# jianzhnie/ScaleRL

Hardware: NVIDIA H100
Metric: learner_frames_per_sec (higher is better)
Workload: dtype bf16

## Files before the change

scalerl_b200/csrc/encoder.cu:

```cuda
#include "encoder_problems.cuh"
#include "tma_problems.cuh"
#include "res_problems.cuh"
#include "enc_fused.cuh"
#include "kernels.h"
#include <stdio.h>
#include <stdlib.h>

namespace srl {

constexpr int PACK_BLOCKS_FK = 256, PACK_BLOCKS_FD = 256, PACK_BLOCKS_CONV = 288;
SRL_DEVINL void pack_store(bf16* __restrict__ out, bf16* __restrict__ out_lo, int64_t i, float v) {
  const bf16 hi = __float2bfloat16_rn(v);
  out[i] = hi;
  if (out_lo) out_lo[i] = __float2bfloat16_rn(v - __bfloat162float(hi));
}
SRL_DEVINL void pack_store2(bf16* __restrict__ out, bf16* __restrict__ out_lo, int64_t i, float v0, float v1) {
  const bf16 h0 = __float2bfloat16_rn(v0), h1 = __float2bfloat16_rn(v1);
  *reinterpret_cast<uint32_t*>(out + i) = pack_bf16x2(v0, v1);
  if (out_lo) *reinterpret_cast<uint32_t*>(out_lo + i) = pack_bf16x2(v0 - __bfloat162float(h0), v1 - __bfloat162float(h1));
}
__global__ void __launch_bounds__(256) pack_weights_kernel(ParamPtrs p, bf16* __restrict__ out, bf16* __restrict__ out_lo, int skip_w1k) {
  pdl_wait(2);
  __shared__ __align__(16) float tile[64 * 99];
  const int t = threadIdx.x, b = blockIdx.x;
  if (b < PACK_BLOCKS_FK) {
    const float4* src = reinterpret_cast<const float4*>(p.wf + (size_t)(2 * b) * 3136);
    float4 v[7];
#pragma unroll
    for (int u = 0; u < 7; ++u) { const int q = t + 256 * u; if (q < 1568) v[u] = __ldg(src + q); }
#pragma unroll
    for (int u = 0; u < 7; ++u) { const int q = t + 256 * u; if (q < 1568) *reinterpret_cast<float4*>(tile + 4 * q) = v[u]; }
    __syncthreads();
#pragma unroll 4
    for (int pp = t; pp < 2 * 1568; pp += 256) {
      const int r = pp >= 1568, k = 2 * (pp - r * 1568), hw = k >> 6, c = k & 63;
      const float* row = tile + r * 3136;
      pack_store2(out, out_lo, WPack::WFK + (int64_t)(2 * b + r) * 3136 + k, row[c * 49 + hw], row[(c + 1) * 49 + hw]);
    }
  } else if (b < PACK_BLOCKS_FK + PACK_BLOCKS_FD) {
    const int bb = b - PACK_BLOCKS_FK, j0 = (bb & 7) * 64, c0 = (bb >> 3) * 2;
    float2 v[13];
#pragma unroll
    for (int u = 0; u < 13; ++u) {
      const int q = t + 256 * u, jj = q / 49, e = q - jj * 49;
      if (q < 64 * 49) v[u] = __ldg(reinterpret_cast<const float2*>(p.wf + (size_t)(j0 + jj) * 3136 + c0 * 49 + 2 * e));
    }
#pragma unroll
    for (int u = 0; u < 13; ++u) {
      const int q = t + 256 * u, jj = q / 49, e = q - jj * 49;
      if (q < 64 * 49) { tile[jj * 99 + 2 * e] = v[u].x; tile[jj * 99 + 2 * e + 1] = v[u].y; }
    }
    __syncthreads();
    const int lane = t & 31, warp = t >> 5;
    for (int kk = warp; kk < 98; kk += 8) {
      const int cc = kk >= 49, hw = kk - cc * 49;
      pack_store2(out, out_lo, WPack::WFD + (int64_t)(hw * 64 + c0 + cc) * 512 + j0 + 2 * lane, tile[(2 * lane) * 99 + kk], tile[(2 * lane + 1) * 99 + kk]);
    }
  } else {
    const int bb = b - PACK_BLOCKS_FK - PACK_BLOCKS_FD;
    constexpr int64_t NCONV = WPack::WFK + (WPack::TOTAL - WPack::W3D);
    for (int64_t n = (int64_t)bb * 256 + t; n < NCONV; n += (int64_t)PACK_BLOCKS_CONV * 256) {
      const int64_t i = n < WPack::WFK ? n : n - WPack::WFK + WPack::W3D;
      float v;
      if (i < WPack::W2K) {
        if (skip_w1k) continue;
        const int e = (int)(i - WPack::W1K), co = e >> 8, k = e & 255, tap = k >> 6, q = k & 63;
        const int c = q >> 4, dy = (q >> 2) & 3, dx = q & 3, kh = 4 * (tap >> 1) + dy, kw = 4 * (tap & 1) + dx;
        v = p.w1[co * 256 + c * 64 + kh * 8 + kw];
      } else if (i < WPack::W3K) {
        const int e = (int)(i - WPack::W2K), co = e >> 9, k = e & 511, tap = k >> 5, c = k & 31;
        v = p.w2[((co * 32 + c) << 4) + tap];
      } else if (i < WPack::WFK) {
        const int e = (int)(i - WPack::W3K), co = e / 576, k = e - co * 576, tap = k >> 6, c = k & 63;
        v = p.w3[(co * 64 + c) * 9 + tap];
      } else if (i < WPack::W2D) {
        const int e = (int)(i - WPack::W3D), c = e / 576, k = e - c * 576, tap = k >> 6, co = k & 63;
        v = p.w3[(co * 64 + c) * 9 + tap];
      } else {
        const int e = (int)(i - WPack::W2D), cls = e >> 13, r = e & 8191, c = r >> 8, k = r & 255, tt = k >> 6, co = k & 63;
        const int kh = (cls >> 1) + 2 * (tt >> 1), kw = (cls & 1) + 2 * (tt & 1);
        v = p.w2[((co * 32 + c) << 4) + kh * 4 + kw];
      }
      pack_store(out, out_lo, i, v);
    }
  }
}

__global__ void __launch_bounds__(352) obs_s2d_kernel(const uint8_t* __restrict__ obs, bf16* __restrict__ xs, int frame_blocks,
                                                      const float* __restrict__ w1, bf16* __restrict__ w1k, bf16* __restrict__ w1k_lo) {
  pdl_wait(1);
  pdl_launch();
  if ((int)blockIdx.x >= frame_blocks) {
    const int e = ((int)blockIdx.x - frame_blocks) * 352 + (int)threadIdx.x;
    if (e < 32 * 256 && w1k) {
      const int co = e >> 8, k = e & 255, tap = k >> 6, q = k & 63;
      const int c = q >> 4, dy = (q >> 2) & 3, dx = q & 3, kh = 4 * (tap >> 1) + dy, kw = 4 * (tap & 1) + dx;
      pack_store(w1k, w1k_lo, e, __ldg(w1 + co * 256 + c * 64 + kh * 8 + kw));
    }
    return;
  }
  __shared__ uint32_t tile[21][16][21];
  const int n = blockIdx.x;
  const int t = threadIdx.x;
  if (t < 336) {
    const int g = t / 21, X = t - g * 21;
    const uint8_t* src = obs + (size_t)n * 28224 + (g >> 2) * 7056 + (g & 3) * 84;
#pragma unroll
    for (int y = 0; y < 21; ++y) tile[y][g][X] = __ldg(reinterpret_cast<const uint32_t*>(src + y * 336) + X);
  }
  __syncthreads();
  if (t < 336) {
    const int X = t >> 4, g = t & 15;
#pragma unroll
    for (int y = 0; y < 21; ++y) {
      const uint32_t w = tile[y][g][X];
      const float f0 = __uint_as_float(__byte_perm(w, 0x4B000000u, 0x7540)) - 8388608.f;
      const float f1 = __uint_as_float(__byte_perm(w, 0x4B000000u, 0x7541)) - 8388608.f;
      const float f2 = __uint_as_float(__byte_perm(w, 0x4B000000u, 0x7542)) - 8388608.f;
      const float f3 = __uint_as_float(__byte_perm(w, 0x4B000000u, 0x7543)) - 8388608.f;
      *reinterpret_cast<uint2*>(xs + (((size_t)n * 21 + y) * 21 + X) * 64 + g * 4) = make_uint2(pack_bf16x2(f0, f1), pack_bf16x2(f2, f3));
    }
  }
}

__global__ void __launch_bounds__(256) a3_transpose_kernel(const bf16* __restrict__ a3, bf16* __restrict__ a3t) {
  pdl_wait(53);
  __shared__ __align__(16) uint16_t tile[49 * 66];
  const int n = blockIdx.x, t = threadIdx.x;
  const uint4* src = reinterpret_cast<const uint4*>(a3 + (size_t)n * 3136);
  for (int q = t; q < 392; q += 256) {
    const uint4 v = __ldg(src + q);
    uint32_t* d = reinterpret_cast<uint32_t*>(tile + (q >> 3) * 66 + (q & 7) * 8);
    d[0] = v.x; d[1] = v.y; d[2] = v.z; d[3] = v.w;
  }
  __syncthreads();
  uint32_t* dst = reinterpret_cast<uint32_t*>(a3t + (size_t)n * 3136);
  for (int pp = t; pp < 1568; pp += 256) {
    const int o = 2 * pp, c0 = o / 49, h0 = o - c0 * 49, o1 = o + 1, c1 = o1 / 49, h1 = o1 - c1 * 49;
    dst[pp] = (uint32_t)tile[h0 * 66 + c0] | ((uint32_t)tile[h1 * 66 + c1] << 16);
  }
}
SRL_KSTAMP_SETTER(kstamp_set_encoder)

cudaError_t launch_a3_transpose(const bf16* a3, bf16* a3t, int frames, cudaStream_t st) {
  if (frames <= 0) return cudaSuccess;
  a3_transpose_kernel<<<frames, 256, 0, st>>>(a3, a3t);
  return cudaGetLastError();
}

cudaError_t launch_pack_weights(const ParamPtrs& p, bf16* wpack, cudaStream_t st, bf16* wpack_lo, bool skip_w1k) {
  pack_weights_kernel<<<PACK_BLOCKS_FK + PACK_BLOCKS_FD + PACK_BLOCKS_CONV, 256, 0, st>>>(p, wpack, wpack_lo, skip_w1k ? 1 : 0);
  return cudaGetLastError();
}

#define SRL_TRY(x) do { cudaError_t e_ = (x); if (e_ != cudaSuccess) return e_; } while (0)

static inline int cdiv(int a, int b) { return (a + b - 1) / b; }

typedef CUresult (*EncodeTiledFn)(CUtensorMap*, CUtensorMapDataType, cuuint32_t, void*, const cuuint64_t*, const cuuint64_t*,
                                  const cuuint32_t*, const cuuint32_t*, CUtensorMapInterleave, CUtensorMapSwizzle,
                                  CUtensorMapL2promotion, CUtensorMapFloatOOBfill);

static EncodeTiledFn encode_fn() {
  static EncodeTiledFn fn = nullptr;
  if (!fn) {
    void* f = nullptr;
    cudaDriverEntryPointQueryResult q;
    if (cudaGetDriverEntryPoint("cuTensorMapEncodeTiled", &f, cudaEnableDefault, &q) == cudaSuccess && q == cudaDriverEntryPointSuccess)
      fn = reinterpret_cast<EncodeTiledFn>(f);
  }
  return fn;
}

bool make_map(CUtensorMap* m, const void* base, int rank, const uint64_t* dims, const uint64_t* strides_elems, const uint32_t* box,
              bool swizzle64) {
  EncodeTiledFn fn = encode_fn();
  if (!fn) return false;
  cuuint64_t gd[5], gs[4];
  cuuint32_t bx[5], es[5];
  for (int i = 0; i < rank; ++i) { gd[i] = dims[i]; bx[i] = box[i]; es[i] = 1; }
  for (int i = 0; i + 1 < rank; ++i) gs[i] = strides_elems[i] * 2;
  return fn(m, CU_TENSOR_MAP_DATA_TYPE_BFLOAT16, (cuuint32_t)rank, const_cast<void*>(base), gd, gs, bx, es, CU_TENSOR_MAP_INTERLEAVE_NONE,
            swizzle64 ? CU_TENSOR_MAP_SWIZZLE_64B : CU_TENSOR_MAP_SWIZZLE_128B, CU_TENSOR_MAP_L2_PROMOTION_L2_128B,
            CU_TENSOR_MAP_FLOAT_OOB_FILL_NONE) == CUDA_SUCCESS;
}

struct MapBuilder {
  const char* failed = nullptr;
  bool lo = false, failed_lo = false;
  void operator()(CUtensorMap* m, const void* base, uint64_t inner, uint64_t rows, uint32_t box_inner, uint32_t box_rows, const char* name,
                  bool swizzle64 = false) {
    const uint64_t d[2] = {inner, rows}, s[1] = {inner};
    const uint32_t bx[2] = {box_inner, box_rows};
    if (!failed && !make_map(m, base, 2, d, s, bx, swizzle64)) { failed = name; failed_lo = lo; }
  }
};

static void build_operand_maps(MapBuilder& mk, const OperandTensors& b, uint64_t nf, uint64_t nb, OperandMaps* M) {
  mk(&M->a1p0_w, b.a1, 64, nf * 100, 64, RConv2Fwd::WROWS, "a1p0_w");
  mk(&M->a1p1_w, b.a1 + (size_t)nf * 100 * 64, 64, nf * 100, 64, RConv2Fwd::WROWS, "a1p1_w");
  mk(&M->a2_w, b.a2, 64, nf * 81, 64, RConv3Fwd::WROWS, "a2_w");
  mk(&M->da3g_w, b.da3, 64, nb * 81, 64, RConv3Dgrad::WROWS, "da3g_w");
  mk(&M->da3g_b, b.da3, 64, nb * 81, 64, 128, "da3g_b");
  mk(&M->da2g_w, b.da2, 64, nb * 100, 64, RConv2Dgrad::WROWS, "da2g_w");
  mk(&M->da2g_b, b.da2, 64, nb * 100, 64, 128, "da2g_b");
  mk(&M->da1g_b, b.da1, 32, nb * 441, 32, 128, "da1g_b", true);
  mk(&M->a3m128, b.a3, 3136, nf, 64, 128, "a3m128");
  mk(&M->a3m64, b.a3, 3136, nf, 64, 64, "a3m64");
  mk(&M->dhm128, b.dh, 512, nb, 64, 128, "dhm128");
  mk(&M->dhm64, b.dh, 512, nb, 64, 64, "dhm64");
  const bf16* w = b.wpack;
  mk(&M->w1k, w + WPack::W1K, 256, 32, 64, 32, "w1k");
  mk(&M->w2k, w + WPack::W2K, 512, 64, 64, 64, "w2k");
  mk(&M->w3k, w + WPack::W3K, 576, 64, 64, 64, "w3k");
  mk(&M->wfk, w + WPack::WFK, 3136, 512, 64, 64, "wfk");
  mk(&M->wfd, w + WPack::WFD, 512, 3136, 64, 64, "wfd");
  mk(&M->w3d, w + WPack::W3D, 576, 64, 64, 64, "w3d");
  mk(&M->w2d, w + WPack::W2D, 256, 128, 64, 128, "w2d");
}

cudaError_t build_tma_maps(const EncoderBuffers& b, int NF, int NB, TmaMaps* M, const char** why) {
  static_assert(RConv1Wgrad::WROWS == RConv1Fwd::WROWS && RConv2Wgrad::WROWS == RConv2Fwd::WROWS && RConv3Wgrad::WROWS == RConv3Fwd::WROWS,
                "forward and wgrad share the window maps");
  const uint64_t nf = NF, nb = NB;
  MapBuilder mk;
  mk(&M->xs_w, b.xs, 64, nf * 441, 64, RConv1Fwd::WROWS, "xs_w");
  mk(&M->a3tm64, b.a3t, 3136, nf, 64, 64, "a3tm64");
  build_operand_maps(mk, b.hi, nf, nb, &M->hi);
  mk.lo = true;
  if (b.lo.wpack) build_operand_maps(mk, b.lo, nf, nb, &M->lo);
  M->valid = !mk.failed;
  if (mk.failed && why) {
    static thread_local char name[32];
    snprintf(name, sizeof(name), "%s%s", mk.failed, mk.failed_lo ? "_lo" : "");
    *why = name;
  }
  return mk.failed ? cudaErrorInvalidValue : cudaSuccess;
}

static cudaError_t launch_s2d(const uint8_t* obs, int frames, bf16* xs, cudaStream_t st, const float* w1, bf16* w1k, bf16* w1k_lo) {
  constexpr int WB = (32 * 256 + 351) / 352;
  SRL_TRY(launch_chain(obs_s2d_kernel, dim3(frames + WB), dim3(352), 0, st, obs, xs, frames, w1, w1k, w1k_lo));
  return cudaGetLastError();
}

static int sm_count() {
  static const int n = [] { int d = 0, v = 0; cudaGetDevice(&d); cudaDeviceGetAttribute(&v, cudaDevAttrMultiProcessorCount, d); return v > 0 ? v : 132; }();
  return n;
}
static int persistent_ctas() {
  static int v = 0;
  if (!v) {
    const char* e = getenv("SRL_PERSISTENT_CTAS");
    v = e ? atoi(e) : sm_count();
    if (v < 16 || v > sm_count()) v = sm_count();
  }
  return v;
}
#define kPersistentCtas persistent_ctas()
static int bwd_ctas() {
  static const int v = [] { const char* e = getenv("SRL_BWD_CTAS"); int x = e ? atoi(e) : 0; return x < 16 || x > sm_count() ? 0 : x; }();
  return v ? v : persistent_ctas() - persistent_ctas() / 9;
}
static int side_wgrad_ctas() {
  static const int v = [] { const char* e = getenv("SRL_WGRAD_CTAS"); int x = e ? atoi(e) : 64; return x < 8 || x > sm_count() ? 64 : x; }();
  return v;
}

struct WgradReduce3 {
  static constexpr int KID = 0, CO = 64, BIAS = 64, PART = WSP_W3, NR = 18, ROW_GROUPS = 32;
  static constexpr bool FRAMES_U8 = false;
  SRL_DEVINL static int row(int rg, int i) { return (i % 9) * 64 + 2 * rg + i / 9; }
};
struct WgradReduce2 {
  static constexpr int KID = 0, CO = 64, BIAS = 64, PART = WSP_W2, NR = 16, ROW_GROUPS = 32;
  static constexpr bool FRAMES_U8 = false;
  SRL_DEVINL static int row(int rg, int i) { return (i >> 2) * 128 + (i & 3) * 32 + rg; }
};
struct WgradReduce1 {
  static constexpr int KID = 51, CO = 32, BIAS = 32, PART = WSP_W1, NR = 16, ROW_GROUPS = 16;
  static constexpr bool FRAMES_U8 = true;
  SRL_DEVINL static int row(int rg, int i) {
    const int c = rg >> 2, kh2 = (rg >> 1) & 1, dy = 2 * (rg & 1) + (i >> 3), kw = i & 7;
    return kh2 * 128 + (kw >> 2) * 64 + c * 16 + dy * 4 + (kw & 3);
  }
};
template <class L>
__global__ void __launch_bounds__(L::NR * 8) conv_wgrad_reduce_kernel(const float* __restrict__ part, int n, float* __restrict__ g,
                                                                       float* __restrict__ db) {
  constexpr int CG = L::CO / 8, TILES = L::ROW_GROUPS * CG;
  static_assert(L::BIAS <= 8 * L::NR, "the bias block fits the tile's threads and shared memory");
  extern __shared__ __align__(16) float stage[];
  pdl_wait(L::KID);
  pdl_launch();
  const int t = threadIdx.x, rg = blockIdx.x / CG, co0 = (blockIdx.x % CG) * 8;
  const bool bias = blockIdx.x == TILES;
  const int per = bias ? L::BIAS / 4 : 2 * L::NR;
  for (int k = t; k < n * per; k += L::NR * 8) {
    const int c = k / per, q = k - c * per;
    const float* src = part + (size_t)c * L::PART + (bias ? L::PART - L::BIAS + 4 * q : L::row(rg, q >> 1) * L::CO + co0 + 4 * (q & 1));
    asm volatile("cp.async.cg.shared.global [%0], [%1], 16;" ::"r"(smem_u32(stage + 4 * k)), "l"(src) : "memory");
  }
  asm volatile("cp.async.wait_all;" ::: "memory");
  __syncthreads();
  const int w = bias ? L::BIAS : 8 * L::NR;
  if (t >= w) return;
  float s = 0.f;
  for (int c = 0; c < n; ++c) s += stage[c * w + t];
  if (bias) db[t] += s;
  else g[(size_t)(co0 + (t & 7)) * (L::ROW_GROUPS * L::NR) + L::NR * rg + (t >> 3)] = L::FRAMES_U8 ? s * (1.0f / 255.0f) : s;
}

template <class L>
static cudaError_t launch_wgrad_reduce(const float* part, int n, float* g, float* db, cudaStream_t st) {
  static PerDeviceOnce once;
  SRL_TRY(ensure_max_dynamic_smem(once, conv_wgrad_reduce_kernel<L>, WG_PART_CTAS * L::NR * 32));
  static const int greatest = [] { int lo = 0, hi = 0; return cudaDeviceGetStreamPriorityRange(&lo, &hi) == cudaSuccess ? hi : 0; }();
  cudaLaunchConfig_t cfg = {};
  cfg.gridDim = dim3(L::ROW_GROUPS * (L::CO / 8) + 1); cfg.blockDim = dim3(L::NR * 8); cfg.dynamicSmemBytes = (size_t)n * L::NR * 32; cfg.stream = st;
  cudaLaunchAttribute attr[1];
  attr[0].id = cudaLaunchAttributePriority;
  attr[0].val.priority = greatest;
  cfg.attrs = attr; cfg.numAttrs = 1;
  return cudaLaunchKernelEx(&cfg, conv_wgrad_reduce_kernel<L>, part, n, g, db);
}

cudaError_t encoder_forward(const uint8_t* obs, int frames, const ParamPtrs& p, const EncoderBuffers& buf, const TmaMaps& maps, int mode,
                            const StepStreams& S, bool fused_front) {
  if (frames <= 0) return cudaSuccess;
  if ((mode != 0 && mode != 1) || !maps.valid) return cudaErrorInvalidValue;
  const int sp = mode;
  if (sp && !buf.lo.wpack) return cudaErrorInvalidValue;
  const cudaStream_t st = S.main;
  if (fused_front && !sp && (reinterpret_cast<uintptr_t>(obs) & 15) == 0) {
    EncFusedParams q{obs, p.w1, p.b1, p.w2, p.b2, buf.xs, buf.hi.a1, buf.hi.a2, frames, buf.NF};
    S.b(PS_ENC_FUSED); SRL_TRY(enc_fused_fwd_launch(q, kPersistentCtas, st)); S.e(PS_ENC_FUSED);
    SRL_TRY(S.join(LANE_PACK));
  } else {
  S.b(PS_S2D); SRL_TRY(launch_s2d(obs, frames, buf.xs, st, p.w1, buf.hi.wpack + WPack::W1K, sp ? buf.lo.wpack + WPack::W1K : nullptr)); S.e(PS_S2D);
  { RConv1Fwd::Params q{maps.xs_w, maps.hi.w1k, maps.lo.w1k, p.b1, buf.hi.a1, buf.lo.a1, frames, buf.NF};
    S.b(PS_CONV1_FWD); SRL_TRY(res_fwd_launch<RConv1Fwd>(q, cdiv(frames * 441, 128), kPersistentCtas, st, sp)); S.e(PS_CONV1_FWD); }
  SRL_TRY(S.join(LANE_PACK));
  { RConv2Fwd::Params q{maps.hi.a1p0_w, maps.hi.a1p1_w, maps.hi.w2k, maps.lo.a1p0_w, maps.lo.a1p1_w, maps.lo.w2k, p.b2, buf.hi.a2, buf.lo.a2, frames};
    S.b(PS_CONV2_FWD); SRL_TRY(res_fwd_launch<RConv2Fwd>(q, cdiv(frames * 100, 128), kPersistentCtas, st, sp)); S.e(PS_CONV2_FWD); }
  }
  { RConv3Fwd::Params q{maps.hi.a2_w, maps.hi.w3k, maps.lo.a2_w, maps.lo.w3k, p.b3, buf.hi.a3, buf.lo.a3, frames};
    S.b(PS_CONV3_FWD); SRL_TRY(res_fwd_launch<RConv3Fwd>(q, cdiv(frames * 81, 128), kPersistentCtas, st, sp)); S.e(PS_CONV3_FWD); }
  { TFcFwd::Params q{maps.hi.a3m128, maps.hi.wfk, maps.lo.a3m128, maps.lo.wfk, buf.hpart, frames};
    static_assert(TFcFwd::SPLITS == FC_SPLITS, "split count");
    S.b(PS_FC_FWD);
    if (sp) SRL_TRY((igemm_tma_launch<TFcFwd, 1>(q, dim3(cdiv(frames, 128), 8 * FC_SPLITS), st)));
    else SRL_TRY((igemm_tma_launch<TFcFwd, 0>(q, dim3(cdiv(frames, 128), 8 * FC_SPLITS), st)));
    S.e(PS_FC_FWD); }
  return cudaSuccess;
}

cudaError_t encoder_backward(int frames, const EncoderBuffers& buf, const ParamPtrs& g, const TmaMaps& maps, int mode,
                             const StepStreams& S, BwdParts parts, bool a3t_done) {
  if (frames <= 0) return cudaSuccess;
  if ((mode != 0 && mode != 1) || !maps.valid) return cudaErrorInvalidValue;
  const int sp = mode;
  if (sp && !buf.lo.wpack) return cudaErrorInvalidValue;
  const bool do_fc = parts & BWD_FC, do_conv = parts & BWD_CONV;
  const cudaStream_t st = S.main, s1 = S.lane(LANE_FC_WGRAD), s2 = S.lane(LANE_CONV3_WGRAD), s3 = S.lane(LANE_CONV2_WGRAD);
  if (do_fc) {
    SRL_TRY(S.fork(LANE_FC_WGRAD));
    { const bool native = !sp && buf.a3t != nullptr;
      S.b(PS_FC_WGRAD);
      if (native) {
        if (!a3t_done) SRL_TRY(launch_a3_transpose(buf.hi.a3, buf.a3t, frames, s1));
        TFcWgradN::Params q{maps.hi.dhm64, maps.a3tm64, g.wf, g.bf, frames};
        SRL_TRY((igemm_tma_launch<TFcWgradN, 0>(q, dim3(1, 4 * (TFcWgradN::NCT + 1)), s1)));
      } else {
        TFcWgrad::Params q{maps.hi.dhm64, maps.hi.a3m64, maps.lo.dhm64, maps.lo.a3m64, g.wf, g.bf, frames};
        if (sp) SRL_TRY((igemm_tma_launch<TFcWgrad, 1>(q, dim3(1, 4 * 50), s1))); else SRL_TRY((igemm_tma_launch<TFcWgrad, 0>(q, dim3(1, 4 * 50), s1)));
      }
      S.e(PS_FC_WGRAD); }
    { TFcDgrad::Params q{maps.hi.dhm128, maps.hi.wfd, maps.lo.dhm128, maps.lo.wfd, buf.hi.a3, buf.hi.da3, buf.lo.da3, frames};
      S.b(PS_FC_DGRAD);
      if (sp) SRL_TRY((igemm_tma_launch<TFcDgrad, 1>(q, dim3(cdiv(frames, 128), 49), st))); else SRL_TRY((igemm_tma_launch<TFcDgrad, 0>(q, dim3(cdiv(frames, 128), 49), st)));
      S.e(PS_FC_DGRAD); }
    if (!do_conv) SRL_TRY(S.join(LANE_FC_WGRAD));
  }
  if (!do_conv) return cudaSuccess;
  SRL_TRY(S.fork(LANE_CONV3_WGRAD));
  float* part3 = buf.wgrad_part;
  float* part2 = part3 + (size_t)WG_PART_CTAS * WSP_W3;
  float* part1 = part2 + (size_t)WG_PART_CTAS * WSP_W2;
  int n3 = 0, n2 = 0, n1 = 0;
  { RConv3Wgrad::Params q{maps.hi.a2_w, maps.hi.da3g_b, maps.lo.a2_w, maps.lo.da3g_b, part3, frames * 81, 0};
    S.b(PS_CONV3_WGRAD); SRL_TRY(res_wgrad_launch<RConv3Wgrad>(q, side_wgrad_ctas(), s2, &n3, sp)); S.e(PS_CONV3_WGRAD); }
  if (!S.collapsed) SRL_TRY(launch_wgrad_reduce<WgradReduce3>(part3, n3, g.w3, g.b3, s2));
  { RConv3Dgrad::Params q{maps.hi.da3g_w, maps.hi.w3d, maps.lo.da3g_w, maps.lo.w3d, buf.hi.a2, buf.hi.da2, buf.lo.da2, frames};
    S.b(PS_CONV3_DGRAD); SRL_TRY(res_fwd_launch<RConv3Dgrad>(q, cdiv(frames * 81, 128), bwd_ctas(), st, sp)); S.e(PS_CONV3_DGRAD); }
  SRL_TRY(S.fork(LANE_CONV2_WGRAD));
  { RConv2Wgrad::Params q{maps.hi.a1p0_w, maps.hi.a1p1_w, maps.hi.da2g_b, maps.lo.a1p0_w, maps.lo.a1p1_w, maps.lo.da2g_b, part2, frames * 100, 0};
    S.b(PS_CONV2_WGRAD); SRL_TRY(res_wgrad_launch<RConv2Wgrad>(q, side_wgrad_ctas(), s3, &n2, sp)); S.e(PS_CONV2_WGRAD); }
  if (!S.collapsed) SRL_TRY(launch_wgrad_reduce<WgradReduce2>(part2, n2, g.w2, g.b2, s3));
  { RConv2Dgrad::Params q{maps.hi.da2g_w, maps.hi.w2d, maps.lo.da2g_w, maps.lo.w2d, buf.hi.a1, buf.hi.da1, buf.lo.da1, frames, buf.NF};
    S.b(PS_CONV2_DGRAD); SRL_TRY(res_fwd_launch<RConv2Dgrad>(q, cdiv(frames * 100, 128), bwd_ctas(), st, sp)); S.e(PS_CONV2_DGRAD); }
  { RConv1Wgrad::Params q{maps.xs_w, maps.hi.da1g_b, maps.lo.da1g_b, part1, frames * 441, 0};
    S.b(PS_CONV1_WGRAD); SRL_TRY(res_wgrad_launch<RConv1Wgrad>(q, bwd_ctas(), st, &n1, sp)); S.e(PS_CONV1_WGRAD); }
  S.b(PS_WGRAD_FINALIZE);
  if (S.collapsed) {
    SRL_TRY(launch_wgrad_reduce<WgradReduce3>(part3, n3, g.w3, g.b3, st));
    SRL_TRY(launch_wgrad_reduce<WgradReduce2>(part2, n2, g.w2, g.b2, st));
  }
  SRL_TRY(launch_wgrad_reduce<WgradReduce1>(part1, n1, g.w1, g.b1, st));
  S.e(PS_WGRAD_FINALIZE);
  if (do_fc) SRL_TRY(S.join(LANE_FC_WGRAD));
  SRL_TRY(S.join(LANE_CONV3_WGRAD));
  SRL_TRY(S.join(LANE_CONV2_WGRAD));
  return cudaSuccess;
}

}
```

scalerl_b200/csrc/tma_problems.cuh:

```cuda
#pragma once
#include "igemm_tma.cuh"
#include "encoder_problems.cuh"

namespace srl {

#define SRL_TMAP alignas(64) CUtensorMap

struct TFcFwd {
  static constexpr int KID = 31;
  static constexpr bool PREFETCH = false;
  static constexpr int BN = 64, STAGES = 4, SPLITS = 4;
  static constexpr bool A_MN = false, B_MN = false, ZERO_INIT = false;
  static constexpr int KROWS = 64;
  struct Params { SRL_TMAP a3m; SRL_TMAP w; SRL_TMAP a3m_lo; SRL_TMAP w_lo; float* out; int M; };
  SRL_DEVINL static void prefetch(const Params& p) { tma_prefetch_desc(&p.a3m); tma_prefetch_desc(&p.w); }
  SRL_DEVINL static int kb_begin(int split) { return (49 * split) / SPLITS; }
  SRL_DEVINL static void issue_split(const Params& p, int tm, int ty, int kb, uint8_t* st, int a_bytes, int half, uint64_t* bar) {
    const int k = (kb_begin(ty % SPLITS) + kb) * 64;
    mbar_arrive_expect_tx(bar, 2 * (128 * 128 + 64 * 128));
    tma_load_2d(st, &p.a3m, bar, k, tm * 128);
    tma_load_2d(st + a_bytes, &p.w, bar, k, (ty / SPLITS) * 64);
    tma_load_2d(st + half, &p.a3m_lo, bar, k, tm * 128);
    tma_load_2d(st + half + a_bytes, &p.w_lo, bar, k, (ty / SPLITS) * 64);
  }
  template <int SPLIT>
  SRL_DEVINL static void epilogue16(const Params& p, int tm, int ty, int row, int c0, float (&v)[16]) { epilogue16(p, tm, ty, row, c0, v); }
  SRL_DEVINL static int num_kblocks(const Params&, int, int ty) { const int sp = ty % SPLITS; return kb_begin(sp + 1) - kb_begin(sp); }
  SRL_DEVINL static void issue(const Params& p, int tm, int ty, int kb, uint8_t* sA, uint8_t* sB, uint64_t* bar) {
    const int k = (kb_begin(ty % SPLITS) + kb) * 64;
    mbar_arrive_expect_tx(bar, 128 * 128 + 64 * 128);
    tma_load_2d(sA, &p.a3m, bar, k, tm * 128);
    tma_load_2d(sB, &p.w, bar, k, (ty / SPLITS) * 64);
  }
  SRL_DEVINL static void epilogue16(const Params& p, int tm, int ty, int row, int c0, float (&v)[16]) {
    const int m = tm * 128 + row;
    if (m >= p.M) return;
    float4* o = reinterpret_cast<float4*>(p.out + ((size_t)(ty % SPLITS) * p.M + m) * 512 + (ty / SPLITS) * 64 + c0);
#pragma unroll
    for (int j = 0; j < 4; ++j) o[j] = make_float4(v[4 * j], v[4 * j + 1], v[4 * j + 2], v[4 * j + 3]);
  }
};

struct TFcDgrad {
  static constexpr int KID = 32;
  static constexpr bool PREFETCH = true;
  static constexpr int BN = 64, STAGES = 4;
  static constexpr bool A_MN = false, B_MN = false, ZERO_INIT = false;
  static constexpr int KROWS = 64;
  struct Params { SRL_TMAP dhm; SRL_TMAP w; SRL_TMAP dhm_lo; SRL_TMAP w_lo; const bf16* a3; bf16* da3; bf16* da3_lo; int M; };
  SRL_DEVINL static void prefetch(const Params& p) { tma_prefetch_desc(&p.dhm); tma_prefetch_desc(&p.w); }
  SRL_DEVINL static int num_kblocks(const Params&, int, int) { return 8; }
  SRL_DEVINL static void issue_split(const Params& p, int tm, int ty, int kb, uint8_t* st, int a_bytes, int half, uint64_t* bar) {
    mbar_arrive_expect_tx(bar, 2 * (128 * 128 + 64 * 128));
    tma_load_2d(st, &p.dhm, bar, kb * 64, tm * 128);
    tma_load_2d(st + a_bytes, &p.w, bar, kb * 64, ty * 64);
    tma_load_2d(st + half, &p.dhm_lo, bar, kb * 64, tm * 128);
    tma_load_2d(st + half + a_bytes, &p.w_lo, bar, kb * 64, ty * 64);
  }
  SRL_DEVINL static void issue(const Params& p, int tm, int ty, int kb, uint8_t* sA, uint8_t* sB, uint64_t* bar) {
    mbar_arrive_expect_tx(bar, 128 * 128 + 64 * 128);
    tma_load_2d(sA, &p.dhm, bar, kb * 64, tm * 128);
    tma_load_2d(sB, &p.w, bar, kb * 64, ty * 64);
  }
  SRL_DEVINL static void prefetch16(const Params& p, int tm, int ty, int row, int c0, uint4 (&mk)[2]) {
    const int m = tm * 128 + row;
    if (m < p.M) ld_mask16(p.a3 + (size_t)m * 3136 + ty * 64 + c0, mk);
  }
  SRL_DEVINL static void epilogue16(const Params& p, int tm, int ty, int row, int c0, float (&v)[16], const uint4 (&mk)[2]) {
    epilogue16<0>(p, tm, ty, row, c0, v, mk);
  }
  template <int SPLIT>
  SRL_DEVINL static void epilogue16(const Params& p, int tm, int ty, int row, int c0, float (&v)[16], const uint4 (&mk)[2]) {
    const int m = tm * 128 + row;
    if (m >= p.M) return;
    relu_mask16_pre(mk, v);
    const size_t o = ((size_t)m * 81 + (ty / 7) * 9 + ty % 7) * 64 + c0;
    store_bf16x16(p.da3 + o, v);
    if constexpr (SPLIT) {
      float r[16];
#pragma unroll
      for (int j = 0; j < 16; ++j) r[j] = v[j] - __bfloat162float(__float2bfloat16_rn(v[j]));
      store_bf16x16(p.da3_lo + o, r);
    }
  }
};

SRL_DEVINL void fill_ones(uint8_t* dst, int bytes, int tid) {
  uint4* q = reinterpret_cast<uint4*>(dst);
  for (int i = tid; i < bytes / 16; i += IGT_THREADS) q[i] = make_uint4(0x3F803F80u, 0x3F803F80u, 0x3F803F80u, 0x3F803F80u);
}

struct TFcWgrad {
  static constexpr int KID = 33;
  static constexpr bool PREFETCH = false;
  static constexpr int BN = 64, STAGES = 4, KROWS = 64;
  static constexpr bool A_MN = true, B_MN = true, ZERO_INIT = true;
  struct Params { SRL_TMAP dhm; SRL_TMAP a3m; SRL_TMAP dhm_lo; SRL_TMAP a3m_lo; float* dw; float* db; int M; };
  SRL_DEVINL static void prefetch(const Params& p) { tma_prefetch_desc(&p.dhm); tma_prefetch_desc(&p.a3m); }
  SRL_DEVINL static void issue_split(const Params& p, int, int ty, int kb, uint8_t* st, int a_bytes, int half, uint64_t* bar) {
    const int hw = ty >> 2, j0 = (ty & 3) * 128;
    mbar_arrive_expect_tx(bar, (hw < 49 ? 6 : 4) * 64 * 128);
    tma_load_2d(st, &p.dhm, bar, j0, kb * 64);
    tma_load_2d(st + KROWS * 128, &p.dhm, bar, j0 + 64, kb * 64);
    tma_load_2d(st + half, &p.dhm_lo, bar, j0, kb * 64);
    tma_load_2d(st + half + KROWS * 128, &p.dhm_lo, bar, j0 + 64, kb * 64);
    if (hw < 49) {
      tma_load_2d(st + a_bytes, &p.a3m, bar, hw * 64, kb * 64);
      tma_load_2d(st + half + a_bytes, &p.a3m_lo, bar, hw * 64, kb * 64);
    }
  }
  template <int SPLIT>
  SRL_DEVINL static void epilogue16(const Params& p, int tm, int ty, int row, int c0, float (&v)[16]) { epilogue16(p, tm, ty, row, c0, v); }
  SRL_DEVINL static bool zero_cta(int) { return true; }
  SRL_DEVINL static int num_kblocks(const Params& p, int, int) { return (p.M + 63) >> 6; }
  SRL_DEVINL static void init_smem(const Params&, int, int ty, uint8_t* stage, int tid) {
    if ((ty >> 2) == 49) fill_ones(stage + 2 * KROWS * 128, KROWS * 128, tid);
  }
  SRL_DEVINL static void issue(const Params& p, int, int ty, int kb, uint8_t* sA, uint8_t* sB, uint64_t* bar) {
    const int hw = ty >> 2, j0 = (ty & 3) * 128;
    mbar_arrive_expect_tx(bar, (hw < 49 ? 3 : 2) * 64 * 128);
    tma_load_2d(sA, &p.dhm, bar, j0, kb * 64);
    tma_load_2d(sA + KROWS * 128, &p.dhm, bar, j0 + 64, kb * 64);
    if (hw < 49) tma_load_2d(sB, &p.a3m, bar, hw * 64, kb * 64);
  }
  SRL_DEVINL static void epilogue16(const Params& p, int, int ty, int row, int c0, float (&v)[16]) {
    const int j = (ty & 3) * 128 + row, hw = ty >> 2;
    if (hw < 49) {
#pragma unroll
      for (int jj = 0; jj < 16; ++jj) p.dw[(size_t)j * 3136 + (c0 + jj) * 49 + hw] = v[jj];
    } else if (c0 == 0) {
      p.db[j] = v[0];
    }
  }
};

struct TFcWgradN {
  static constexpr int KID = 36;
  static constexpr bool PREFETCH = false;
  static constexpr int BN = 256, STAGES = 4, KROWS = 64, NCT = 13;
  static constexpr bool A_MN = true, B_MN = true, ZERO_INIT = true;
  struct Params { SRL_TMAP dhm; SRL_TMAP a3tm; float* dw; float* db; int M; };
  SRL_DEVINL static void prefetch(const Params& p) { tma_prefetch_desc(&p.dhm); tma_prefetch_desc(&p.a3tm); }
  SRL_DEVINL static bool zero_cta(int ty) { return (ty >> 2) == NCT; }
  SRL_DEVINL static int num_kblocks(const Params& p, int, int) { return (p.M + 63) >> 6; }
  SRL_DEVINL static void init_smem(const Params&, int, int ty, uint8_t* stage, int tid) {
    if ((ty >> 2) == NCT) fill_ones(stage + 2 * KROWS * 128, KROWS * 128, tid);
  }
  SRL_DEVINL static void issue(const Params& p, int, int ty, int kb, uint8_t* sA, uint8_t* sB, uint64_t* bar) {
    const int ct = ty >> 2, j0 = (ty & 3) * 128;
    const int nb = ct < NCT ? (ct == NCT - 1 ? 1 : 4) : 0;
    mbar_arrive_expect_tx(bar, (2 + nb) * 64 * 128);
    tma_load_2d(sA, &p.dhm, bar, j0, kb * 64);
    tma_load_2d(sA + KROWS * 128, &p.dhm, bar, j0 + 64, kb * 64);
    for (int q = 0; q < nb; ++q) tma_load_2d(sB + q * KROWS * 128, &p.a3tm, bar, ct * 256 + q * 64, kb * 64);
  }
  SRL_DEVINL static void epilogue16(const Params& p, int, int ty, int row, int c0, float (&v)[16]) {
    const int j = (ty & 3) * 128 + row, ct = ty >> 2, col = ct * 256 + c0;
    if (ct < NCT) {
      if (col < 3136) {
        float4* d = reinterpret_cast<float4*>(p.dw + (size_t)j * 3136 + col);
#pragma unroll
        for (int q = 0; q < 4; ++q) d[q] = make_float4(v[4 * q], v[4 * q + 1], v[4 * q + 2], v[4 * q + 3]);
      }
    } else if (c0 == 0) {
      p.db[j] = v[0];
    }
  }
};

}
```

Before: 2.480 million.

## Retile FC forward, dgrad and wgrad GEMMs to 128-wide N tiles

Widens the N tile of the FC forward and dgrad TMA GEMMs from 64 to 128 columns, so each CTA loads two weight boxes per stage and reuses each activation tile across twice as many outputs. Both launches shrink their grid to match. The native wgrad kernel moves from 256-wide to 128-wide column tiles and folds the bias (ones column) into the last, partially filled tile instead of using a separate CTA group. The aim is less redundant A-operand traffic and no extra bias CTAs, at the cost of different occupancy, more shared memory per stage, and new boundary handling for the ragged last tile.

Result: no change. 2.491 million, median of 6 (+0.4%).

```diff
diff --git a/scalerl_b200/csrc/encoder.cu b/scalerl_b200/csrc/encoder.cu
--- a/scalerl_b200/csrc/encoder.cu
+++ b/scalerl_b200/csrc/encoder.cu
@@ -349,8 +349,8 @@
   { TFcFwd::Params q{maps.hi.a3m128, maps.hi.wfk, maps.lo.a3m128, maps.lo.wfk, buf.hpart, frames};
     static_assert(TFcFwd::SPLITS == FC_SPLITS, "split count");
     S.b(PS_FC_FWD);
-    if (sp) SRL_TRY((igemm_tma_launch<TFcFwd, 1>(q, dim3(cdiv(frames, 128), 8 * FC_SPLITS), st)));
-    else SRL_TRY((igemm_tma_launch<TFcFwd, 0>(q, dim3(cdiv(frames, 128), 8 * FC_SPLITS), st)));
+    const dim3 grid(cdiv(frames, 128), TFcFwd::NT * FC_SPLITS);
+    if (sp) SRL_TRY((igemm_tma_launch<TFcFwd, 1>(q, grid, st))); else SRL_TRY((igemm_tma_launch<TFcFwd, 0>(q, grid, st)));
     S.e(PS_FC_FWD); }
   return cudaSuccess;
 }
@@ -370,7 +370,7 @@
       if (native) {
         if (!a3t_done) SRL_TRY(launch_a3_transpose(buf.hi.a3, buf.a3t, frames, s1));
         TFcWgradN::Params q{maps.hi.dhm64, maps.a3tm64, g.wf, g.bf, frames};
-        SRL_TRY((igemm_tma_launch<TFcWgradN, 0>(q, dim3(1, 4 * (TFcWgradN::NCT + 1)), s1)));
+        SRL_TRY((igemm_tma_launch<TFcWgradN, 0>(q, dim3(1, 4 * TFcWgradN::NCT), s1)));
       } else {
         TFcWgrad::Params q{maps.hi.dhm64, maps.hi.a3m64, maps.lo.dhm64, maps.lo.a3m64, g.wf, g.bf, frames};
         if (sp) SRL_TRY((igemm_tma_launch<TFcWgrad, 1>(q, dim3(1, 4 * 50), s1))); else SRL_TRY((igemm_tma_launch<TFcWgrad, 0>(q, dim3(1, 4 * 50), s1)));
@@ -378,7 +378,8 @@
       S.e(PS_FC_WGRAD); }
     { TFcDgrad::Params q{maps.hi.dhm128, maps.hi.wfd, maps.lo.dhm128, maps.lo.wfd, buf.hi.a3, buf.hi.da3, buf.lo.da3, frames};
       S.b(PS_FC_DGRAD);
-      if (sp) SRL_TRY((igemm_tma_launch<TFcDgrad, 1>(q, dim3(cdiv(frames, 128), 49), st))); else SRL_TRY((igemm_tma_launch<TFcDgrad, 0>(q, dim3(cdiv(frames, 128), 49), st)));
+      const dim3 grid(cdiv(frames, 128), TFcDgrad::NT);
+      if (sp) SRL_TRY((igemm_tma_launch<TFcDgrad, 1>(q, grid, st))); else SRL_TRY((igemm_tma_launch<TFcDgrad, 0>(q, grid, st)));
       S.e(PS_FC_DGRAD); }
     if (!do_conv) SRL_TRY(S.join(LANE_FC_WGRAD));
   }
diff --git a/scalerl_b200/csrc/tma_problems.cuh b/scalerl_b200/csrc/tma_problems.cuh
--- a/scalerl_b200/csrc/tma_problems.cuh
+++ b/scalerl_b200/csrc/tma_problems.cuh
@@ -9,33 +9,36 @@
 struct TFcFwd {
   static constexpr int KID = 31;
   static constexpr bool PREFETCH = false;
-  static constexpr int BN = 64, STAGES = 4, SPLITS = 4;
+  static constexpr int BN = 128, STAGES = 4, SPLITS = 4, NT = 512 / BN;
   static constexpr bool A_MN = false, B_MN = false, ZERO_INIT = false;
   static constexpr int KROWS = 64;
   struct Params { SRL_TMAP a3m; SRL_TMAP w; SRL_TMAP a3m_lo; SRL_TMAP w_lo; float* out; int M; };
   SRL_DEVINL static void prefetch(const Params& p) { tma_prefetch_desc(&p.a3m); tma_prefetch_desc(&p.w); }
   SRL_DEVINL static int kb_begin(int split) { return (49 * split) / SPLITS; }
   SRL_DEVINL static void issue_split(const Params& p, int tm, int ty, int kb, uint8_t* st, int a_bytes, int half, uint64_t* bar) {
-    const int k = (kb_begin(ty % SPLITS) + kb) * 64;
-    mbar_arrive_expect_tx(bar, 2 * (128 * 128 + 64 * 128));
+    const int k = (kb_begin(ty % SPLITS) + kb) * 64, n0 = (ty / SPLITS) * BN;
+    mbar_arrive_expect_tx(bar, 2 * (128 * 128 + BN * 128));
     tma_load_2d(st, &p.a3m, bar, k, tm * 128);
-    tma_load_2d(st + a_bytes, &p.w, bar, k, (ty / SPLITS) * 64);
+    tma_load_2d(st + a_bytes, &p.w, bar, k, n0);
+    tma_load_2d(st + a_bytes + 64 * 128, &p.w, bar, k, n0 + 64);
     tma_load_2d(st + half, &p.a3m_lo, bar, k, tm * 128);
-    tma_load_2d(st + half + a_bytes, &p.w_lo, bar, k, (ty / SPLITS) * 64);
+    tma_load_2d(st + half + a_bytes, &p.w_lo, bar, k, n0);
+    tma_load_2d(st + half + a_bytes + 64 * 128, &p.w_lo, bar, k, n0 + 64);
   }
   template <int SPLIT>
   SRL_DEVINL static void epilogue16(const Params& p, int tm, int ty, int row, int c0, float (&v)[16]) { epilogue16(p, tm, ty, row, c0, v); }
   SRL_DEVINL static int num_kblocks(const Params&, int, int ty) { const int sp = ty % SPLITS; return kb_begin(sp + 1) - kb_begin(sp); }
   SRL_DEVINL static void issue(const Params& p, int tm, int ty, int kb, uint8_t* sA, uint8_t* sB, uint64_t* bar) {
-    const int k = (kb_begin(ty % SPLITS) + kb) * 64;
-    mbar_arrive_expect_tx(bar, 128 * 128 + 64 * 128);
+    const int k = (kb_begin(ty % SPLITS) + kb) * 64, n0 = (ty / SPLITS) * BN;
+    mbar_arrive_expect_tx(bar, 128 * 128 + BN * 128);
     tma_load_2d(sA, &p.a3m, bar, k, tm * 128);
-    tma_load_2d(sB, &p.w, bar, k, (ty / SPLITS) * 64);
+    tma_load_2d(sB, &p.w, bar, k, n0);
+    tma_load_2d(sB + 64 * 128, &p.w, bar, k, n0 + 64);
   }
   SRL_DEVINL static void epilogue16(const Params& p, int tm, int ty, int row, int c0, float (&v)[16]) {
     const int m = tm * 128 + row;
     if (m >= p.M) return;
-    float4* o = reinterpret_cast<float4*>(p.out + ((size_t)(ty % SPLITS) * p.M + m) * 512 + (ty / SPLITS) * 64 + c0);
+    float4* o = reinterpret_cast<float4*>(p.out + ((size_t)(ty % SPLITS) * p.M + m) * 512 + (ty / SPLITS) * BN + c0);
 #pragma unroll
     for (int j = 0; j < 4; ++j) o[j] = make_float4(v[4 * j], v[4 * j + 1], v[4 * j + 2], v[4 * j + 3]);
   }
@@ -44,37 +47,43 @@
 struct TFcDgrad {
   static constexpr int KID = 32;
   static constexpr bool PREFETCH = true;
-  static constexpr int BN = 64, STAGES = 4;
+  static constexpr int BN = 128, STAGES = 4, NT = (3136 + BN - 1) / BN;
+  SRL_DEVINL static bool two_boxes(int ty) { return ty * BN + 64 < 3136; }
   static constexpr bool A_MN = false, B_MN = false, ZERO_INIT = false;
   static constexpr int KROWS = 64;
   struct Params { SRL_TMAP dhm; SRL_TMAP w; SRL_TMAP dhm_lo; SRL_TMAP w_lo; const bf16* a3; bf16* da3; bf16* da3_lo; int M; };
   SRL_DEVINL static void prefetch(const Params& p) { tma_prefetch_desc(&p.dhm); tma_prefetch_desc(&p.w); }
   SRL_DEVINL static int num_kblocks(const Params&, int, int) { return 8; }
   SRL_DEVINL static void issue_split(const Params& p, int tm, int ty, int kb, uint8_t* st, int a_bytes, int half, uint64_t* bar) {
-    mbar_arrive_expect_tx(bar, 2 * (128 * 128 + 64 * 128));
+    const bool two = two_boxes(ty);
+    mbar_arrive_expect_tx(bar, 2 * (128 * 128 + (two ? 2 : 1) * 64 * 128));
     tma_load_2d(st, &p.dhm, bar, kb * 64, tm * 128);
-    tma_load_2d(st + a_bytes, &p.w, bar, kb * 64, ty * 64);
+    tma_load_2d(st + a_bytes, &p.w, bar, kb * 64, ty * BN);
+    if (two) tma_load_2d(st + a_bytes + 64 * 128, &p.w, bar, kb * 64, ty * BN + 64);
     tma_load_2d(st + half, &p.dhm_lo, bar, kb * 64, tm * 128);
-    tma_load_2d(st + half + a_bytes, &p.w_lo, bar, kb * 64, ty * 64);
+    tma_load_2d(st + half + a_bytes, &p.w_lo, bar, kb * 64, ty * BN);
+    if (two) tma_load_2d(st + half + a_bytes + 64 * 128, &p.w_lo, bar, kb * 64, ty * BN + 64);
   }
   SRL_DEVINL static void issue(const Params& p, int tm, int ty, int kb, uint8_t* sA, uint8_t* sB, uint64_t* bar) {
-    mbar_arrive_expect_tx(bar, 128 * 128 + 64 * 128);
+    const bool two = two_boxes(ty);
+    mbar_arrive_expect_tx(bar, 128 * 128 + (two ? 2 : 1) * 64 * 128);
     tma_load_2d(sA, &p.dhm, bar, kb * 64, tm * 128);
-    tma_load_2d(sB, &p.w, bar, kb * 64, ty * 64);
+    tma_load_2d(sB, &p.w, bar, kb * 64, ty * BN);
+    if (two) tma_load_2d(sB + 64 * 128, &p.w, bar, kb * 64, ty * BN + 64);
   }
   SRL_DEVINL static void prefetch16(const Params& p, int tm, int ty, int row, int c0, uint4 (&mk)[2]) {
-    const int m = tm * 128 + row;
-    if (m < p.M) ld_mask16(p.a3 + (size_t)m * 3136 + ty * 64 + c0, mk);
+    const int m = tm * 128 + row, col = ty * BN + c0;
+    if (m < p.M && col < 3136) ld_mask16(p.a3 + (size_t)m * 3136 + col, mk);
   }
   SRL_DEVINL static void epilogue16(const Params& p, int tm, int ty, int row, int c0, float (&v)[16], const uint4 (&mk)[2]) {
     epilogue16<0>(p, tm, ty, row, c0, v, mk);
   }
   template <int SPLIT>
   SRL_DEVINL static void epilogue16(const Params& p, int tm, int ty, int row, int c0, float (&v)[16], const uint4 (&mk)[2]) {
-    const int m = tm * 128 + row;
-    if (m >= p.M) return;
+    const int m = tm * 128 + row, col = ty * BN + c0, hw = col >> 6;
+    if (m >= p.M || col >= 3136) return;
     relu_mask16_pre(mk, v);
-    const size_t o = ((size_t)m * 81 + (ty / 7) * 9 + ty % 7) * 64 + c0;
+    const size_t o = ((size_t)m * 81 + (hw / 7) * 9 + hw % 7) * 64 + (col & 63);
     store_bf16x16(p.da3 + o, v);
     if constexpr (SPLIT) {
       float r[16];
@@ -137,32 +146,30 @@
 struct TFcWgradN {
   static constexpr int KID = 36;
   static constexpr bool PREFETCH = false;
-  static constexpr int BN = 256, STAGES = 4, KROWS = 64, NCT = 13;
+  static constexpr int BN = 128, STAGES = 4, KROWS = 64, NCT = (3136 + BN - 1) / BN;
   static constexpr bool A_MN = true, B_MN = true, ZERO_INIT = true;
   struct Params { SRL_TMAP dhm; SRL_TMAP a3tm; float* dw; float* db; int M; };
   SRL_DEVINL static void prefetch(const Params& p) { tma_prefetch_desc(&p.dhm); tma_prefetch_desc(&p.a3tm); }
-  SRL_DEVINL static bool zero_cta(int ty) { return (ty >> 2) == NCT; }
+  SRL_DEVINL static bool zero_cta(int) { return false; }
   SRL_DEVINL static int num_kblocks(const Params& p, int, int) { return (p.M + 63) >> 6; }
   SRL_DEVINL static void init_smem(const Params&, int, int ty, uint8_t* stage, int tid) {
-    if ((ty >> 2) == NCT) fill_ones(stage + 2 * KROWS * 128, KROWS * 128, tid);
+    if ((ty >> 2) == NCT - 1) fill_ones(stage + 3 * KROWS * 128, KROWS * 128, tid);
   }
   SRL_DEVINL static void issue(const Params& p, int, int ty, int kb, uint8_t* sA, uint8_t* sB, uint64_t* bar) {
     const int ct = ty >> 2, j0 = (ty & 3) * 128;
-    const int nb = ct < NCT ? (ct == NCT - 1 ? 1 : 4) : 0;
+    const int nb = ct == NCT - 1 ? 1 : 2;
     mbar_arrive_expect_tx(bar, (2 + nb) * 64 * 128);
     tma_load_2d(sA, &p.dhm, bar, j0, kb * 64);
     tma_load_2d(sA + KROWS * 128, &p.dhm, bar, j0 + 64, kb * 64);
-    for (int q = 0; q < nb; ++q) tma_load_2d(sB + q * KROWS * 128, &p.a3tm, bar, ct * 256 + q * 64, kb * 64);
+    for (int q = 0; q < nb; ++q) tma_load_2d(sB + q * KROWS * 128, &p.a3tm, bar, ct * BN + q * 64, kb * 64);
   }
   SRL_DEVINL static void epilogue16(const Params& p, int, int ty, int row, int c0, float (&v)[16]) {
-    const int j = (ty & 3) * 128 + row, ct = ty >> 2, col = ct * 256 + c0;
-    if (ct < NCT) {
-      if (col < 3136) {
-        float4* d = reinterpret_cast<float4*>(p.dw + (size_t)j * 3136 + col);
+    const int j = (ty & 3) * 128 + row, col = (ty >> 2) * BN + c0;
+    if (col < 3136) {
+      float4* d = reinterpret_cast<float4*>(p.dw + (size_t)j * 3136 + col);
 #pragma unroll
-        for (int q = 0; q < 4; ++q) d[q] = make_float4(v[4 * q], v[4 * q + 1], v[4 * q + 2], v[4 * q + 3]);
-      }
-    } else if (c0 == 0) {
+      for (int q = 0; q < 4; ++q) d[q] = make_float4(v[4 * q], v[4 * q + 1], v[4 * q + 2], v[4 * q + 3]);
+    } else if (col == 3136) {
       p.db[j] = v[0];
     }
   }
```

## Retile FC forward, dgrad and wgrad GEMMs to 128-wide N tiles

Applied to the files above, without the earlier changes.

The FC forward and FC dgrad TMA GEMMs move from 64-wide to 128-wide N tiles, loading several 64-row weight blocks per stage. Dgrad now covers two output pixels per CTA, with a ragged last tile. The native FC wgrad moves from 256 to 128 columns and puts the bias ones-column into the spare 64-column block of the last tile, removing the separate bias CTA. The aim is better reuse of the A operand and fewer redundant A loads and CTAs, at the cost of more shared memory per stage, fewer CTAs for wave balance, and extra edge handling.

Result: no change. 2.512 million before, 2.510 million after (median of 6 runs) (-0.1%).

```diff
diff --git a/scalerl_b200/csrc/encoder.cu b/scalerl_b200/csrc/encoder.cu
--- a/scalerl_b200/csrc/encoder.cu
+++ b/scalerl_b200/csrc/encoder.cu
@@ -349,8 +349,8 @@
   { TFcFwd::Params q{maps.hi.a3m128, maps.hi.wfk, maps.lo.a3m128, maps.lo.wfk, buf.hpart, frames};
     static_assert(TFcFwd::SPLITS == FC_SPLITS, "split count");
     S.b(PS_FC_FWD);
-    if (sp) SRL_TRY((igemm_tma_launch<TFcFwd, 1>(q, dim3(cdiv(frames, 128), 8 * FC_SPLITS), st)));
-    else SRL_TRY((igemm_tma_launch<TFcFwd, 0>(q, dim3(cdiv(frames, 128), 8 * FC_SPLITS), st)));
+    if (sp) SRL_TRY((igemm_tma_launch<TFcFwd, 1>(q, dim3(cdiv(frames, 128), TFcFwd::NT * FC_SPLITS), st)));
+    else SRL_TRY((igemm_tma_launch<TFcFwd, 0>(q, dim3(cdiv(frames, 128), TFcFwd::NT * FC_SPLITS), st)));
     S.e(PS_FC_FWD); }
   return cudaSuccess;
 }
@@ -370,7 +370,7 @@
       if (native) {
         if (!a3t_done) SRL_TRY(launch_a3_transpose(buf.hi.a3, buf.a3t, frames, s1));
         TFcWgradN::Params q{maps.hi.dhm64, maps.a3tm64, g.wf, g.bf, frames};
-        SRL_TRY((igemm_tma_launch<TFcWgradN, 0>(q, dim3(1, 4 * (TFcWgradN::NCT + 1)), s1)));
+        SRL_TRY((igemm_tma_launch<TFcWgradN, 0>(q, dim3(1, 4 * TFcWgradN::NCT), s1)));
       } else {
         TFcWgrad::Params q{maps.hi.dhm64, maps.hi.a3m64, maps.lo.dhm64, maps.lo.a3m64, g.wf, g.bf, frames};
         if (sp) SRL_TRY((igemm_tma_launch<TFcWgrad, 1>(q, dim3(1, 4 * 50), s1))); else SRL_TRY((igemm_tma_launch<TFcWgrad, 0>(q, dim3(1, 4 * 50), s1)));
@@ -378,7 +378,7 @@
       S.e(PS_FC_WGRAD); }
     { TFcDgrad::Params q{maps.hi.dhm128, maps.hi.wfd, maps.lo.dhm128, maps.lo.wfd, buf.hi.a3, buf.hi.da3, buf.lo.da3, frames};
       S.b(PS_FC_DGRAD);
-      if (sp) SRL_TRY((igemm_tma_launch<TFcDgrad, 1>(q, dim3(cdiv(frames, 128), 49), st))); else SRL_TRY((igemm_tma_launch<TFcDgrad, 0>(q, dim3(cdiv(frames, 128), 49), st)));
+      if (sp) SRL_TRY((igemm_tma_launch<TFcDgrad, 1>(q, dim3(cdiv(frames, 128), TFcDgrad::NT), st))); else SRL_TRY((igemm_tma_launch<TFcDgrad, 0>(q, dim3(cdiv(frames, 128), TFcDgrad::NT), st)));
       S.e(PS_FC_DGRAD); }
     if (!do_conv) SRL_TRY(S.join(LANE_FC_WGRAD));
   }
diff --git a/scalerl_b200/csrc/tma_problems.cuh b/scalerl_b200/csrc/tma_problems.cuh
--- a/scalerl_b200/csrc/tma_problems.cuh
+++ b/scalerl_b200/csrc/tma_problems.cuh
@@ -6,10 +6,14 @@
 
 #define SRL_TMAP alignas(64) CUtensorMap
 
+SRL_DEVINL void tma_load_rows(uint8_t* dst, const CUtensorMap* m, uint64_t* bar, int k, int row0, int blocks) {
+  for (int q = 0; q < blocks; ++q) tma_load_2d(dst + q * 64 * 128, m, bar, k, row0 + q * 64);
+}
+
 struct TFcFwd {
   static constexpr int KID = 31;
   static constexpr bool PREFETCH = false;
-  static constexpr int BN = 64, STAGES = 4, SPLITS = 4;
+  static constexpr int BN = 128, STAGES = 4, SPLITS = 4, NT = 512 / BN;
   static constexpr bool A_MN = false, B_MN = false, ZERO_INIT = false;
   static constexpr int KROWS = 64;
   struct Params { SRL_TMAP a3m; SRL_TMAP w; SRL_TMAP a3m_lo; SRL_TMAP w_lo; float* out; int M; };
@@ -17,25 +21,25 @@
   SRL_DEVINL static int kb_begin(int split) { return (49 * split) / SPLITS; }
   SRL_DEVINL static void issue_split(const Params& p, int tm, int ty, int kb, uint8_t* st, int a_bytes, int half, uint64_t* bar) {
     const int k = (kb_begin(ty % SPLITS) + kb) * 64;
-    mbar_arrive_expect_tx(bar, 2 * (128 * 128 + 64 * 128));
+    mbar_arrive_expect_tx(bar, 2 * (128 * 128 + BN * 128));
     tma_load_2d(st, &p.a3m, bar, k, tm * 128);
-    tma_load_2d(st + a_bytes, &p.w, bar, k, (ty / SPLITS) * 64);
+    tma_load_rows(st + a_bytes, &p.w, bar, k, (ty / SPLITS) * BN, BN / 64);
     tma_load_2d(st + half, &p.a3m_lo, bar, k, tm * 128);
-    tma_load_2d(st + half + a_bytes, &p.w_lo, bar, k, (ty / SPLITS) * 64);
+    tma_load_rows(st + half + a_bytes, &p.w_lo, bar, k, (ty / SPLITS) * BN, BN / 64);
   }
   template <int SPLIT>
   SRL_DEVINL static void epilogue16(const Params& p, int tm, int ty, int row, int c0, float (&v)[16]) { epilogue16(p, tm, ty, row, c0, v); }
   SRL_DEVINL static int num_kblocks(const Params&, int, int ty) { const int sp = ty % SPLITS; return kb_begin(sp + 1) - kb_begin(sp); }
   SRL_DEVINL static void issue(const Params& p, int tm, int ty, int kb, uint8_t* sA, uint8_t* sB, uint64_t* bar) {
     const int k = (kb_begin(ty % SPLITS) + kb) * 64;
-    mbar_arrive_expect_tx(bar, 128 * 128 + 64 * 128);
+    mbar_arrive_expect_tx(bar, 128 * 128 + BN * 128);
     tma_load_2d(sA, &p.a3m, bar, k, tm * 128);
-    tma_load_2d(sB, &p.w, bar, k, (ty / SPLITS) * 64);
+    tma_load_rows(sB, &p.w, bar, k, (ty / SPLITS) * BN, BN / 64);
   }
   SRL_DEVINL static void epilogue16(const Params& p, int tm, int ty, int row, int c0, float (&v)[16]) {
     const int m = tm * 128 + row;
     if (m >= p.M) return;
-    float4* o = reinterpret_cast<float4*>(p.out + ((size_t)(ty % SPLITS) * p.M + m) * 512 + (ty / SPLITS) * 64 + c0);
+    float4* o = reinterpret_cast<float4*>(p.out + ((size_t)(ty % SPLITS) * p.M + m) * 512 + (ty / SPLITS) * BN + c0);
 #pragma unroll
     for (int j = 0; j < 4; ++j) o[j] = make_float4(v[4 * j], v[4 * j + 1], v[4 * j + 2], v[4 * j + 3]);
   }
@@ -44,37 +48,40 @@
 struct TFcDgrad {
   static constexpr int KID = 32;
   static constexpr bool PREFETCH = true;
-  static constexpr int BN = 64, STAGES = 4;
+  static constexpr int BN = 128, STAGES = 4, PIX = BN / 64, NT = (49 + PIX - 1) / PIX;
   static constexpr bool A_MN = false, B_MN = false, ZERO_INIT = false;
   static constexpr int KROWS = 64;
   struct Params { SRL_TMAP dhm; SRL_TMAP w; SRL_TMAP dhm_lo; SRL_TMAP w_lo; const bf16* a3; bf16* da3; bf16* da3_lo; int M; };
   SRL_DEVINL static void prefetch(const Params& p) { tma_prefetch_desc(&p.dhm); tma_prefetch_desc(&p.w); }
   SRL_DEVINL static int num_kblocks(const Params&, int, int) { return 8; }
+  SRL_DEVINL static int pixels(int ty) { return min(PIX, 49 - ty * PIX); }
   SRL_DEVINL static void issue_split(const Params& p, int tm, int ty, int kb, uint8_t* st, int a_bytes, int half, uint64_t* bar) {
-    mbar_arrive_expect_tx(bar, 2 * (128 * 128 + 64 * 128));
+    const int nb = pixels(ty);
+    mbar_arrive_expect_tx(bar, 2 * (128 + nb * 64) * 128);
     tma_load_2d(st, &p.dhm, bar, kb * 64, tm * 128);
-    tma_load_2d(st + a_bytes, &p.w, bar, kb * 64, ty * 64);
+    tma_load_rows(st + a_bytes, &p.w, bar, kb * 64, ty * BN, nb);
     tma_load_2d(st + half, &p.dhm_lo, bar, kb * 64, tm * 128);
-    tma_load_2d(st + half + a_bytes, &p.w_lo, bar, kb * 64, ty * 64);
+    tma_load_rows(st + half + a_bytes, &p.w_lo, bar, kb * 64, ty * BN, nb);
   }
   SRL_DEVINL static void issue(const Params& p, int tm, int ty, int kb, uint8_t* sA, uint8_t* sB, uint64_t* bar) {
-    mbar_arrive_expect_tx(bar, 128 * 128 + 64 * 128);
+    const int nb = pixels(ty);
+    mbar_arrive_expect_tx(bar, (128 + nb * 64) * 128);
     tma_load_2d(sA, &p.dhm, bar, kb * 64, tm * 128);
-    tma_load_2d(sB, &p.w, bar, kb * 64, ty * 64);
+    tma_load_rows(sB, &p.w, bar, kb * 64, ty * BN, nb);
   }
   SRL_DEVINL static void prefetch16(const Params& p, int tm, int ty, int row, int c0, uint4 (&mk)[2]) {
     const int m = tm * 128 + row;
-    if (m < p.M) ld_mask16(p.a3 + (size_t)m * 3136 + ty * 64 + c0, mk);
+    if (m < p.M && ty * PIX + c0 / 64 < 49) ld_mask16(p.a3 + (size_t)m * 3136 + ty * BN + c0, mk);
   }
   SRL_DEVINL static void epilogue16(const Params& p, int tm, int ty, int row, int c0, float (&v)[16], const uint4 (&mk)[2]) {
     epilogue16<0>(p, tm, ty, row, c0, v, mk);
   }
   template <int SPLIT>
   SRL_DEVINL static void epilogue16(const Params& p, int tm, int ty, int row, int c0, float (&v)[16], const uint4 (&mk)[2]) {
-    const int m = tm * 128 + row;
-    if (m >= p.M) return;
+    const int m = tm * 128 + row, hw = ty * PIX + c0 / 64;
+    if (m >= p.M || hw >= 49) return;
     relu_mask16_pre(mk, v);
-    const size_t o = ((size_t)m * 81 + (ty / 7) * 9 + ty % 7) * 64 + c0;
+    const size_t o = ((size_t)m * 81 + (hw / 7) * 9 + hw % 7) * 64 + c0 % 64;
     store_bf16x16(p.da3 + o, v);
     if constexpr (SPLIT) {
       float r[16];
@@ -137,32 +144,31 @@
 struct TFcWgradN {
   static constexpr int KID = 36;
   static constexpr bool PREFETCH = false;
-  static constexpr int BN = 256, STAGES = 4, KROWS = 64, NCT = 13;
+  static constexpr int BN = 128, STAGES = 4, KROWS = 64, NCT = (3136 + BN - 1) / BN;
+  static_assert(3136 % BN == 64, "the last column tile has a spare 64-column block for the ones");
   static constexpr bool A_MN = true, B_MN = true, ZERO_INIT = true;
   struct Params { SRL_TMAP dhm; SRL_TMAP a3tm; float* dw; float* db; int M; };
   SRL_DEVINL static void prefetch(const Params& p) { tma_prefetch_desc(&p.dhm); tma_prefetch_desc(&p.a3tm); }
-  SRL_DEVINL static bool zero_cta(int ty) { return (ty >> 2) == NCT; }
+  SRL_DEVINL static bool zero_cta(int) { return false; }
   SRL_DEVINL static int num_kblocks(const Params& p, int, int) { return (p.M + 63) >> 6; }
   SRL_DEVINL static void init_smem(const Params&, int, int ty, uint8_t* stage, int tid) {
-    if ((ty >> 2) == NCT) fill_ones(stage + 2 * KROWS * 128, KROWS * 128, tid);
+    if ((ty >> 2) == NCT - 1) fill_ones(stage + 3 * KROWS * 128, KROWS * 128, tid);
   }
   SRL_DEVINL static void issue(const Params& p, int, int ty, int kb, uint8_t* sA, uint8_t* sB, uint64_t* bar) {
     const int ct = ty >> 2, j0 = (ty & 3) * 128;
-    const int nb = ct < NCT ? (ct == NCT - 1 ? 1 : 4) : 0;
+    const int nb = ct == NCT - 1 ? 1 : BN / 64;
     mbar_arrive_expect_tx(bar, (2 + nb) * 64 * 128);
     tma_load_2d(sA, &p.dhm, bar, j0, kb * 64);
     tma_load_2d(sA + KROWS * 128, &p.dhm, bar, j0 + 64, kb * 64);
-    for (int q = 0; q < nb; ++q) tma_load_2d(sB + q * KROWS * 128, &p.a3tm, bar, ct * 256 + q * 64, kb * 64);
+    for (int q = 0; q < nb; ++q) tma_load_2d(sB + q * KROWS * 128, &p.a3tm, bar, ct * BN + q * 64, kb * 64);
   }
   SRL_DEVINL static void epilogue16(const Params& p, int, int ty, int row, int c0, float (&v)[16]) {
-    const int j = (ty & 3) * 128 + row, ct = ty >> 2, col = ct * 256 + c0;
-    if (ct < NCT) {
-      if (col < 3136) {
-        float4* d = reinterpret_cast<float4*>(p.dw + (size_t)j * 3136 + col);
+    const int j = (ty & 3) * 128 + row, col = (ty >> 2) * BN + c0;
+    if (col < 3136) {
+      float4* d = reinterpret_cast<float4*>(p.dw + (size_t)j * 3136 + col);
 #pragma unroll
-        for (int q = 0; q < 4; ++q) d[q] = make_float4(v[4 * q], v[4 * q + 1], v[4 * q + 2], v[4 * q + 3]);
-      }
-    } else if (c0 == 0) {
+      for (int q = 0; q < 4; ++q) d[q] = make_float4(v[4 * q], v[4 * q + 1], v[4 * q + 2], v[4 * q + 3]);
+    } else if (col == 3136) {
       p.db[j] = v[0];
     }
   }
```
